# UBC-AWP/vision-sam3-yolo-lameless

Measured on AMD Instinct MI355X. Metric: frames/sec (whole node) for YOLO+SAM3+DINOv3 feature extraction, 1080p clips, higher is better.
Workload: dtype f16; 1 GPU; BASELINE cfg#5, dense schedule: fused per-frame path on a synthetic 5 s @ 30 fps 1080p clip (150 unique BGR frames resident in HBM): YOLOv8-l detect (letterbox 384x640, NMS, scale_boxes; f16 plan) -> SAM (Hiera-B+ image encoder + FPN at 1024x1024, box-prompted mask decoder, 1080p mask + statistics + contour features) + DINOv3 ViT-L/16 embed (224x224) on EVERY frame; per-frame records packed, gathe; parallelism=one clip per GPU, 1 GPU(s), one gather per step, streams=7

## Files before the change

include/lmx.h:

```cpp
#ifndef LMX_H
#define LMX_H
#include <stdint.h>
#ifdef __cplusplus
extern "C" {
#endif

#define LMX_VERSION 100

#define LMX_OK 0
#define LMX_EINVAL (-1)
#define LMX_EHIP (-2)

typedef void* lmx_stream_t;

int lmx_version(void);
const char* lmx_last_error(void);
int lmx_device_count(void);

enum { LMX_F16 = 0, LMX_F32 = 1 };
enum { LMX_ACT_NONE = 0, LMX_ACT_SILU = 1, LMX_ACT_GELU = 2 , LMX_ACT_RELU = 3,
       LMX_ACT_SWIGLU = 4  };

typedef struct {
  const void* A;
// ... 98 lines not shown
                        int a_off, int A, lmx_stream_t stream);
int lmx_k_scale_boxes(float* boxes, int total, float padx, float pady, float gain, float w, float h,
                      lmx_stream_t stream);

int lmx_k_split3(const float* x, int64_t ldx, int act, const void* res3, int64_t ldr, void* out3, int64_t ldo, int64_t rows,
                 int N, int g, int nsum, int64_t sum_stride, lmx_stream_t stream);
int lmx_k_maxpool5_x3(const void* src3, int64_t lds, void* dst3, int64_t ldd, int n, int H, int W, int C, lmx_stream_t stream);
int lmx_k_stem_conv_x3(const uint8_t* img, const float* w, const float* bias, void* out3, int n, int H, int W, int Cout,
                       lmx_stream_t stream);
int lmx_k_attention_f32(const float* q, int64_t ldq, const float* k, int64_t ldk, const float* v, int64_t ldv, float* o,
                        int64_t ldo, int B, int H, int Tq, int Tk, int hd, float scale, lmx_stream_t stream);
int lmx_k_hyper_mask_f32(const float* up, const float* hyper, float* logits, int n, int G, int C, int act, lmx_stream_t stream);

int lmx_k_pose_gather(const float* raw0, const float* raw1, const float* raw2, int64_t ldk, const int32_t* hw,
                      const float* strides, const int32_t* src, const int32_t* counts, int n, int max_det, int K, int ndim,
                      float padx, float pady, float gain, float w, float h, float* out, lmx_stream_t stream);

int lmx_k_im2col_u8(const uint8_t* img, const float* lut, void* out, int n, int rh, int rw, int IH, int IW, int KH,
                    int KW, int stride, int pad, int64_t ldo, lmx_stream_t stream);
int lmx_k_maxpool2(const void* src, int64_t lds, void* dst, int64_t ldd, int dtype, int n, int H, int W, int C,
                   lmx_stream_t stream);
int lmx_k_cast_f32_f16(const float* src, int64_t lds, void* dst, int64_t ldd, int64_t rows, int cols,
                       lmx_stream_t stream);

int lmx_k_add_bcast(const void* a, int a_dtype, int64_t lda, const float* b, int64_t ldb, int b_rows, void* out,
                    int out_dtype, int64_t ldo, int64_t rows, int D, lmx_stream_t stream);
int lmx_k_prompt_box(const float* boxes, int64_t ldb, float* sparse, int n, double sx, double sy, float S,
                     const float* gauss, const float* corner, int F, lmx_stream_t stream);
int lmx_k_hyper_mask(const void* up, const float* hyper, float* logits, int n, int G, int C, lmx_stream_t stream);
int lmx_k_mask_post(const float* logits, int n, int L, int T, int nh, int nw, int h, int w, uint8_t* mask,
                    int64_t* stats, float* workspace, lmx_stream_t stream);
int lmx_k_prompt_points(const float* points, const int32_t* labels, int Np, const float* boxes, int64_t ldb, float* sparse, int n,
                        double sx, double sy, float S, const float* gauss, const float* point_embed, const float* not_a_point,
                        const float* corner, int F, lmx_stream_t stream);
#define LMX_MASK_EMBED_PARAMS 4684
int lmx_k_mask_embed(const float* mask_input, const void* emb, int emb_dtype, int64_t lde, const float* params, float* keys,
                     int64_t ldk, int n, int G, lmx_stream_t stream);
int lmx_k_hyper_mask_multi(const void* up, const float* hyper, float* logits, int n, int M, int G, int C, lmx_stream_t stream);
int lmx_k_hyper_mask_multi_f32(const float* up, const float* hyper, float* logits, int n, int M, int G, int C, int act,
                               lmx_stream_t stream);
int lmx_k_mask_logits(const float* logits, int n, int L, int T, int nh, int nw, int h, int w, float* out, lmx_stream_t stream);

int lmx_k_mask_score(const float* logits, int n, int L, int T, int nh, int nw, int h, int w, double thr, double off,
                     const int32_t* idx, int64_t* out, lmx_stream_t stream);
int lmx_k_nms_boxes(const float* boxes, int64_t ldb, const float* scores, const uint8_t* valid, int n, double iou, int32_t* keep_out,
                    int32_t* count_out, void* workspace, lmx_stream_t stream);
// ... 15 lines not shown
```

vision-sam3-yolo-lameless_amd/csrc/sam.hip:

```cpp
#include "common.h"

namespace {

inline int grid_for(int64_t total, int block = 256) {
  int64_t g = (total + block - 1) / block;
  if (g > 256 * 8) g = 256 * 8;
  if (g < 1) g = 1;
  return (int)g;
}

template <int KW_T>
__global__ __launch_bounds__(256) void im2col_u8_kernel(const uint8_t* __restrict__ img, const float* __restrict__ lut,
                                                        half_t* __restrict__ out, int n, int rh, int rw, int OH, int OW, int KH,
                                                        int KW_rt, int stride, int pad, int64_t ldo) {
  __shared__ float lut_s[768];
  for (int i = threadIdx.x; i < 768; i += blockDim.x) lut_s[i] = lut[i];
  __syncthreads();
  const int KW = KW_T > 0 ? KW_T : KW_rt;
  const int chunks = (int)(ldo / 8);
  const int K = KH * KW * 3;
  const int64_t total = (int64_t)n * OH * OW * chunks;
  for (int64_t i = (int64_t)blockIdx.x * blockDim.x + threadIdx.x; i < total; i += (int64_t)gridDim.x * blockDim.x) {
    const int ck = (int)(i % chunks);
    const int64_t tok = i / chunks;
// ... 41 lines not shown
#pragma unroll
    for (int e = 0; e < VEC; ++e) {
      T t0 = a0[e] > a1[e] ? a0[e] : a1[e];
      T t1 = a2[e] > a3[e] ? a2[e] : a3[e];
      m[e] = t0 > t1 ? t0 : t1;
    }
    *reinterpret_cast<vec_t*>(dst + p * ldd + c) = m;
  }
}

__global__ __launch_bounds__(256) void cast_kernel(const float* __restrict__ src, int64_t lds, half_t* __restrict__ dst, int64_t ldd,
                                                   int64_t rows, int cols) {
  const int cc = cols / 4;
  const int64_t total = rows * cc;
  for (int64_t i = (int64_t)blockIdx.x * blockDim.x + threadIdx.x; i < total; i += (int64_t)gridDim.x * blockDim.x) {
    const int c = (int)(i % cc) * 4;
    const int64_t r = i / cc;
    const f32x4 v = *reinterpret_cast<const f32x4*>(src + r * lds + c);
    half4_t h = {(half_t)v[0], (half_t)v[1], (half_t)v[2], (half_t)v[3]};
    *reinterpret_cast<half4_t*>(dst + r * ldd + c) = h;
  }
}


template <int IN_DT, int OUT_DT>
__global__ __launch_bounds__(256) void add_bcast_kernel(const void* __restrict__ av, int64_t lda, const float* __restrict__ b,
                                                        int64_t ldb, int b_rows, void* __restrict__ out, int64_t ldo, int64_t rows,
                                                        int D) {
  const int cc = D / 4;
  const int64_t total = rows * cc;
  for (int64_t i = (int64_t)blockIdx.x * blockDim.x + threadIdx.x; i < total; i += (int64_t)gridDim.x * blockDim.x) {
    const int c = (int)(i % cc) * 4;
    const int64_t r = i / cc;
    f32x4 v;
    if (IN_DT == LMX_F32) {
      v = *reinterpret_cast<const f32x4*>(reinterpret_cast<const float*>(av) + r * lda + c);
    } else {
      const half4_t hv = *reinterpret_cast<const half4_t*>(reinterpret_cast<const half_t*>(av) + r * lda + c);
      v = f32x4{(float)hv[0], (float)hv[1], (float)hv[2], (float)hv[3]};
    }
    v += *reinterpret_cast<const f32x4*>(b + (r % b_rows) * ldb + c);
    if (OUT_DT == LMX_F32) {
      *reinterpret_cast<f32x4*>(reinterpret_cast<float*>(out) + r * ldo + c) = v;
    } else {
      half4_t h = {(half_t)v[0], (half_t)v[1], (half_t)v[2], (half_t)v[3]};
      *reinterpret_cast<half4_t*>(reinterpret_cast<half_t*>(out) + r * ldo + c) = h;
// ... 228 lines not shown
    hipLaunchKernelGGL((maxpool2_kernel<half_t, 8>), dim3(grid_for((int64_t)n * (H / 2) * (W / 2) * (C / 8))), dim3(256), 0, st,
                       reinterpret_cast<const half_t*>(src), lds, reinterpret_cast<half_t*>(dst), ldd, n, H, W, C);
  } else if (dtype == LMX_F32) {
    LMX_REQUIRE(C % 4 == 0 && lds % 4 == 0 && ldd % 4 == 0 && aligned16(src) && aligned16(dst), "lmx_k_maxpool2: f32 alignment");
    hipLaunchKernelGGL((maxpool2_kernel<float, 4>), dim3(grid_for((int64_t)n * (H / 2) * (W / 2) * (C / 4))), dim3(256), 0, st,
                       reinterpret_cast<const float*>(src), lds, reinterpret_cast<float*>(dst), ldd, n, H, W, C);
  } else {
    LMX_REQUIRE(false, "lmx_k_maxpool2: dtype %d", dtype);
  }
  return lmx_launch_check("maxpool2_kernel");
}

extern "C" int lmx_k_cast_f32_f16(const float* src, int64_t lds, void* dst, int64_t ldd, int64_t rows, int cols,
                                  lmx_stream_t stream) {
  LMX_REQUIRE(src && dst, "lmx_k_cast_f32_f16: null pointer");
  LMX_REQUIRE(rows > 0 && cols > 0 && cols % 4 == 0 && lds % 4 == 0 && ldd % 4 == 0 && lds >= cols && ldd >= cols,
              "lmx_k_cast_f32_f16: shape");
  LMX_REQUIRE(aligned16(src) && ((((uintptr_t)dst) & 7) == 0), "lmx_k_cast_f32_f16: alignment");
  hipLaunchKernelGGL(cast_kernel, dim3(grid_for(rows * (cols / 4))), dim3(256), 0, reinterpret_cast<hipStream_t>(stream), src, lds,
                     reinterpret_cast<half_t*>(dst), ldd, rows, cols);
  return lmx_launch_check("cast_kernel");
}

extern "C" int lmx_k_prompt_box(const float* boxes, int64_t ldb, float* sparse, int n, double sx, double sy, float S,
                                const float* gauss, const float* corner, int F, lmx_stream_t stream) {
  LMX_REQUIRE(boxes && sparse && gauss && corner && n > 0 && F > 0 && ldb >= 4 && S > 0.f, "lmx_k_prompt_box: arguments");
  hipLaunchKernelGGL(prompt_box_kernel, dim3((n * 2 * F + 255) / 256), dim3(256), 0, reinterpret_cast<hipStream_t>(stream), boxes, ldb,
                     sparse, n, sx, sy, S, gauss, corner, F);
  return lmx_launch_check("prompt_box_kernel");
}

extern "C" int lmx_k_add_bcast(const void* a, int a_dtype, int64_t lda, const float* b, int64_t ldb, int b_rows, void* out,
                               int out_dtype, int64_t ldo, int64_t rows, int D, lmx_stream_t stream) {
  LMX_REQUIRE(a && b && out, "lmx_k_add_bcast: null pointer");
  LMX_REQUIRE(rows > 0 && D > 0 && D % 4 == 0 && b_rows > 0 && lda >= D && ldb >= D && ldo >= D && lda % 4 == 0 && ldb % 4 == 0 &&
                  ldo % 4 == 0, "lmx_k_add_bcast: shape");
  LMX_REQUIRE(((((uintptr_t)a) & (a_dtype == LMX_F32 ? 15 : 7)) == 0) && aligned16(b) &&
                  ((((uintptr_t)out) & (out_dtype == LMX_F32 ? 15 : 7)) == 0), "lmx_k_add_bcast: alignment");
  hipStream_t st = reinterpret_cast<hipStream_t>(stream);
  const int g = grid_for(rows * (D / 4));
  if (a_dtype == LMX_F32 && out_dtype == LMX_F32)
    hipLaunchKernelGGL((add_bcast_kernel<LMX_F32, LMX_F32>), dim3(g), dim3(256), 0, st, a, lda, b, ldb, b_rows, out, ldo, rows, D);
  else if (a_dtype == LMX_F32 && out_dtype == LMX_F16)
    hipLaunchKernelGGL((add_bcast_kernel<LMX_F32, LMX_F16>), dim3(g), dim3(256), 0, st, a, lda, b, ldb, b_rows, out, ldo, rows, D);
  else if (a_dtype == LMX_F16 && out_dtype == LMX_F32)
    hipLaunchKernelGGL((add_bcast_kernel<LMX_F16, LMX_F32>), dim3(g), dim3(256), 0, st, a, lda, b, ldb, b_rows, out, ldo, rows, D);
// ... 59 lines not shown
```

vision-sam3-yolo-lameless_amd/lmx/_lib.py:

```python
import ctypes as C
import os

_HERE = os.path.dirname(os.path.abspath(__file__))
LIB_PATH = os.environ.get("LMX_LIB") or os.path.join(_HERE, "liblmx.so")


class LmxError(RuntimeError):
    pass


class GemmDesc(C.Structure):
    _fields_ = [
        ("A", C.c_void_p), ("W", C.c_void_p), ("bias", C.c_void_p), ("scale", C.c_void_p), ("res", C.c_void_p),
        ("C", C.c_void_p),
        ("lda", C.c_int64), ("ldc", C.c_int64), ("ldr", C.c_int64),
        ("M", C.c_int32), ("N", C.c_int32), ("K", C.c_int32),
        ("act", C.c_int32), ("out_dtype", C.c_int32), ("a_mode", C.c_int32),
        ("H", C.c_int32), ("W_", C.c_int32), ("Cin", C.c_int32), ("conv_stride", C.c_int32),
        ("Ho", C.c_int32), ("Wo", C.c_int32), ("res_rows", C.c_int32), ("a_rep", C.c_int32), ("split_k", C.c_int32), ("split_stride", C.c_int64),
        ("ln_out", C.c_void_p), ("ln_gamma", C.c_void_p), ("ln_beta", C.c_void_p), ("ld_ln", C.c_int64), ("ln_eps", C.c_float),
    ]


class AttnDesc(C.Structure):
# ... 32 lines not shown
    "lmx_k_pil_resize_h": (_I, [_VP, _VP, _I, _I, _I, _I, _VP, _VP, _I, _I, _VP]),
    "lmx_k_pil_resize_v": (_I, [_VP, _VP, _I, _I, _I, _I, _VP, _VP, _I, _VP]),
    "lmx_k_patchify_norm": (_I, [_VP, _VP, _I, _I, _I, _I, _I, _I, _I, _I, _I64, _VP, _VP]),
    "lmx_k_float_resize_patchify": (_I, [_VP, _VP, _I, _I, _I, _I, _I, _I, _I64, _VP, _VP, _I, _VP, _VP, _I, _I, _F, _VP, _I, _VP]),
    "lmx_k_assemble_tokens": (_I, [_VP, _VP, _VP, _VP, _I, _I, _I, _I, _VP]),
    "lmx_k_token_mean": (_I, [_VP, _I, _VP, _I, _I, _I, _VP]),
    "lmx_k_swiglu": (_I, [_VP, _I64, _VP, _I64, _I, _I, _VP]),
    "lmx_nms_workspace_bytes": (_I64, [_I, _I]),
    "lmx_k_nms": (_I, [_VP, _I, _I, _I, _F, _D, _I, _F, _VP, _VP, _VP, _VP, _VP, _VP, _VP]),
    "lmx_k_letterbox": (_I, [_VP, _VP, _I, _I, _I, _I, _I, _I, _I, _I, _I, _VP, _VP, _VP, _VP, _I, _VP]),
    "lmx_k_stem_conv": (_I, [_VP, _VP, _VP, _VP, _I, _I, _I, _I, _VP]),
    "lmx_k_split3": (_I, [_VP, _I64, _I, _VP, _I64, _VP, _I64, _I64, _I, _I, _I, _I64, _VP]),
    "lmx_k_maxpool5_x3": (_I, [_VP, _I64, _VP, _I64, _I, _I, _I, _I, _VP]),
    "lmx_k_stem_conv_x3": (_I, [_VP, _VP, _VP, _VP, _I, _I, _I, _I, _VP]),
    "lmx_k_attention_f32": (_I, [_VP, _I64, _VP, _I64, _VP, _I64, _VP, _I64, _I, _I, _I, _I, _I, _F, _VP]),
    "lmx_k_hyper_mask_f32": (_I, [_VP, _VP, _VP, _I, _I, _I, _I, _VP]),
    "lmx_k_maxpool5": (_I, [_VP, _I64, _VP, _I64, _I, _I, _I, _I, _VP]),
    "lmx_k_upsample2": (_I, [_VP, _I64, _VP, _I64, _I, _I, _I, _I, _VP]),
    "lmx_k_detect_decode": (_I, [_VP, _I64, _VP, _I, _I, _I, _I, _F, _I, _I, _VP]),
    "lmx_k_scale_boxes": (_I, [_VP, _I, _F, _F, _F, _F, _F, _VP]),
    "lmx_k_im2col_u8": (_I, [_VP, _VP, _VP, _I, _I, _I, _I, _I, _I, _I, _I, _I, _I64, _VP]),
    "lmx_k_maxpool2": (_I, [_VP, _I64, _VP, _I64, _I, _I, _I, _I, _I, _VP]),
    "lmx_k_cast_f32_f16": (_I, [_VP, _I64, _VP, _I64, _I64, _I, _VP]),
    "lmx_k_add_bcast": (_I, [_VP, _I, _I64, _VP, _I64, _I, _VP, _I, _I64, _I64, _I, _VP]),
    "lmx_h_mask_features": (_I, [_VP, _I, _I, _VP]),
    "lmx_h_iou_matrix": (_I, [_VP, _I, _VP, _I, _VP]),
    "lmx_h_assign": (_I, [_VP, _I, _I, _VP, _VP]),
    "lmx_contour_workspace_bytes": (_I64, [_I, _I, _I]),
    "lmx_k_contour_features": (_I, [_VP, _I, _I, _I, _VP, _VP, _VP]),
    "lmx_k_prompt_box": (_I, [_VP, _I64, _VP, _I, _D, _D, _F, _VP, _VP, _I, _VP]),
    "lmx_k_hyper_mask": (_I, [_VP, _VP, _VP, _I, _I, _I, _VP]),
    "lmx_k_mask_post": (_I, [_VP, _I, _I, _I, _I, _I, _I, _I, _VP, _VP, _VP, _VP]),
    "lmx_k_prompt_points": (_I, [_VP, _VP, _I, _VP, _I64, _VP, _I, _D, _D, _F, _VP, _VP, _VP, _VP, _I, _VP]),
    "lmx_k_mask_embed": (_I, [_VP, _VP, _I, _I64, _VP, _VP, _I64, _I, _I, _VP]),
    "lmx_k_hyper_mask_multi": (_I, [_VP, _VP, _VP, _I, _I, _I, _I, _VP]),
    "lmx_k_hyper_mask_multi_f32": (_I, [_VP, _VP, _VP, _I, _I, _I, _I, _I, _VP]),
    "lmx_k_mask_logits": (_I, [_VP, _I, _I, _I, _I, _I, _I, _I, _VP, _VP]),
    "lmx_k_mask_score": (_I, [_VP, _I, _I, _I, _I, _I, _I, _I, _D, _D, _VP, _VP, _VP]),
    "lmx_k_nms_boxes": (_I, [_VP, _I64, _VP, _VP, _I, _D, _VP, _VP, _VP, _VP]),
}

_lib = None


def load():
    global _lib
    if _lib is not None:
# ... 21 lines not shown
```

vision-sam3-yolo-lameless_amd/lmx/adapters.py:

```python
from pathlib import Path

import numpy as np
import torch

from . import checkpoints, dino, sam, sam_decoder, yolo
from .graphs import GraphedFn


def _device(device):
    if not torch.cuda.is_available():
        raise RuntimeError("lmx adapters need a GPU (liblmx has no CPU path)")
    return torch.device(device if device is not None else "cuda")


class Boxes:

    def __init__(self, xyxy, conf, cls):
        self.xyxy, self.conf, self.cls = xyxy, conf, cls

    def __len__(self):
        return int(self.xyxy.shape[0])

    def __getitem__(self, i):
        if isinstance(i, int):
# ... 150 lines not shown
    def apply_boxes(self, boxes, original_size):
        return self.apply_coords(np.asarray(boxes).reshape(-1, 2, 2), original_size).reshape(-1, 4)

    def apply_coords_torch(self, coords, original_size):
        old_h, old_w = original_size
        new_h, new_w = self.get_preprocess_shape(old_h, old_w, self.target_length)
        coords = coords.clone().to(torch.float)
        coords[..., 0] = coords[..., 0] * (new_w / old_w)
        coords[..., 1] = coords[..., 1] * (new_h / old_h)
        return coords

    def apply_boxes_torch(self, boxes, original_size):
        return self.apply_coords_torch(boxes.reshape(-1, 2, 2), original_size).reshape(-1, 4)


class LmxSamPredictor:

    def __init__(self, sam_model):
        self.model = sam_model
        self.encoder, self.decoder = sam_model.image_encoder, sam_model.mask_decoder
        self.device = sam_model.device
        self.transform = ResizeLongestSide(self.encoder.cfg.image)
        self.is_image_set = False
        self._g_encode = GraphedFn(lambda f: self.encoder.encode(f)["fpn"][2], clone_outputs=False)
        self._g_decode = {}

    @classmethod
    def from_parts(cls, encoder, decoder):
        m = type("LmxSamParts", (), {})()
        m.image_encoder, m.mask_decoder, m.device, m.cfg = encoder, decoder, encoder.device, encoder.cfg
        return cls(m)

    def reset_image(self):
        self.is_image_set = False
        self.features = None
        self.original_size = self.input_size = None

    def set_image(self, image, image_format="RGB"):
        a = np.asarray(image)
        if a.dtype != np.uint8 or a.ndim != 3 or a.shape[2] != 3:
            raise ValueError(f"set_image expects an HWC uint8 image, got {a.dtype} {a.shape}")
        if image_format not in ("RGB", "BGR"):
            raise ValueError(f"image_format must be 'RGB' or 'BGR', is {image_format}")
        if image_format == "BGR":
            a = a[..., ::-1]
        frames = torch.from_numpy(np.ascontiguousarray(a)[None]).to(self.device)
        self.original_size = tuple(a.shape[:2])
# ... 161 lines not shown
```

vision-sam3-yolo-lameless_amd/lmx/kernels.py:

```python
import ctypes as C
import os
import threading

import torch

from . import _lib
from ._lib import AttnDesc, GemmDesc, LmxError, check

F16, F32 = 0, 1
ACT_NONE, ACT_SILU, ACT_GELU, ACT_RELU, ACT_SWIGLU = 0, 1, 2, 3, 4
_DT = {torch.float16: F16, torch.float32: F32}


_tls = threading.local()


def _stream(dev):
    _tls.dev = dev
    return C.c_void_p(torch.cuda.current_stream(dev).cuda_stream)


def _ptr(t):
    return C.c_void_p(t.data_ptr()) if t is not None else C.c_void_p(0)

# ... 146 lines not shown
    out = torch.empty((n * OH * OW, ldo), dtype=torch.float16, device=img.device)
    check(_lib.load().lmx_k_im2col_u8(_ptr(img), _ptr(lut), _ptr(out), n, rh, rw, IH, IW, KH, KW, stride, pad, ldo,
                                      _stream(dev)), "lmx_k_im2col_u8")
    return out


def maxpool2(x, out):
    dev = _dev(x, out)
    n, H, W, Cc, ps = _nhwc(x, "maxpool2 x")
    no, Ho, Wo, Co, pso = _nhwc(out, "maxpool2 out")
    if (no, Ho, Wo, Co) != (n, H // 2, W // 2, Cc) or x.dtype != out.dtype:
        raise LmxError("maxpool2: shape/dtype mismatch")
    check(_lib.load().lmx_k_maxpool2(_ptr(x), ps, _ptr(out), pso, _DT[x.dtype], n, H, W, Cc, _stream(dev)), "lmx_k_maxpool2")
    return out


def cast_f16(x, out=None):
    dev = _dev(x, out)
    rows, cols, lds = _rows(x, "cast src")
    if out is None:
        out = torch.empty((rows, cols), dtype=torch.float16, device=x.device)
    check(_lib.load().lmx_k_cast_f32_f16(_ptr(x), lds, _ptr(out), out.stride(0), rows, cols, _stream(dev)),
          "lmx_k_cast_f32_f16")
    return out


def _nhwc(t, what):
    if t.dim() != 4 or t.stride(3) != 1:
        raise LmxError(f"{what}: expected NHWC with contiguous channels, got {tuple(t.shape)} / {t.stride()}")
    n, H, W, Cc = t.shape
    ps = t.stride(2)
    if t.stride(1) != W * ps or (n > 1 and t.stride(0) != H * W * ps):
        raise LmxError(f"{what}: not a channel slice of a dense NHWC buffer: strides {t.stride()}")
    return n, H, W, Cc, ps


def split_k_for(px_per_frame, N, K, cin):
    if N < 64 or N % 8 or cin % 32:
        return 1
    tiles1 = -(-px_per_frame // 256) * -(-N // 256)
    nk = K // 64
    s = min(8, nk // 8, 32 // tiles1)
    return s if s >= 2 else 1


def conv3x3(x, w, bias=None, act=ACT_SILU, stride=1, res=None, out=None, scale=None, out_dtype=torch.float16, split_k=1):
# ... 703 lines not shown
        return "fused attention half", rows * (8.0 * D * D + 256.0 * D), rows * D * (8 + (2 if args[0] else 0)), f"hiera_attn8 rows={rows} D={D} ln_inside={int(not args[0])}"
    if name == "lmx_k_hiera_attn4":
        n_, Gh, Gw, D = args[5], args[6], args[7], args[8]
        rows = n_ * Gh * Gw
        return "fused attention half", rows * (8.0 * D * D + 64.0 * D), rows * D * 10, f"hiera_attn4 rows={rows} D={D}"
    if name == "lmx_k_hiera_attn_pool":
        n_, Gh, Gw, Di, Do = args[4], args[5], args[6], args[7], args[8]
        rows = n_ * Gh * Gw
        keys = 64 if Di == 112 else 16
        return "fused attention half", rows * (8.0 * Di * Do + keys * Do + 0.5 * Do * Do), rows * (2 * Di + Do), f"hiera_attn_pool rows={rows} {Di}->{Do}"
    if name == "lmx_k_cast_f32_f16":
        rows, cols = args[4], args[5]
        return "streaming glue", 0.0, 6 * rows * cols, f"cast_f32_f16 rows={rows} cols={cols}"
    if name == "lmx_k_maxpool2":
        dt, n_, H, W, C_ = args[4], args[5], args[6], args[7], args[8]
        esz = 4 if dt == F32 else 2
        return "streaming glue", 0.0, esz * n_ * H * W * C_ * 5 // 4, f"maxpool2 n={n_} H={H} W={W} C={C_} dtype={dt}"
    if name == "lmx_k_upsample2":
        n_, H, W, C_ = args[4], args[5], args[6], args[7]
        return "streaming glue", 0.0, 2 * n_ * H * W * C_ * 5, f"upsample2 n={n_} H={H} W={W} C={C_}"
    if name == "lmx_k_add_bcast":
        a_dt, o_dt, rows, D = args[1], args[7], args[9], args[10]
        return "streaming glue", 0.0, rows * D * ((4 if a_dt == F32 else 2) + (4 if o_dt == F32 else 2)), f"add_bcast rows={rows} D={D}"
    if name == "lmx_k_rope":
        B, T, H, hd = args[2], args[3], args[4], args[5]
        return "streaming glue", 0.0, 2 * 2 * 2 * B * T * H * hd, f"rope B={B} T={T} H={H} hd={hd}"
    return "pre/post-processing and glue", 0.0, None, name


def _install_trace():
    global _raw_lib
    if _raw_lib is not None:
        return
    lib = _raw_lib = _lib.load()

    def make(name, fn):
        def traced(*args):
            if LAUNCH_TRACE is None:
                return fn(*args)
            cls, fl, by, key = _work(name, args)
            st = torch.cuda.current_stream(_tls.dev)
            e0, e1 = torch.cuda.Event(enable_timing=True), torch.cuda.Event(enable_timing=True)
            e0.record(st)
            rc = fn(*args)
            e1.record(st)
            LAUNCH_TRACE.append((cls, key, fl, by, e0, e1))
# ... 36 lines not shown
```

vision-sam3-yolo-lameless_amd/lmx/pipeline.py:

```python
import os

import torch

from . import dino, sam, sam_decoder, yolo
from . import kernels as K

DATA = os.path.join(os.path.dirname(os.path.abspath(__file__)), "data")


def stream_plan(n_chunks, max_streams=4, layout="lanes"):
    if layout not in ("lanes", "rr"):
        raise ValueError(f"stream layout {layout!r}: expected 'lanes' or 'rr'")
    k = max(3, min(2 + n_chunks, int(max_streams)))
    if layout == "rr":
        return k, 0, 1, [(2 + j) % k for j in range(n_chunks)]
    return k, 0, 1, [2 + j % (k - 2) for j in range(n_chunks)]


class FusedExtractor:
    def __init__(self, device="cuda", yolo_scale="l", weight_seeds=(7, 5, 3), yolo_bn=None):
        from . import weights

        self.device = torch.device(device)
        self.serial = bool(os.environ.get("LMX_SERIAL"))
# ... 67 lines not shown
            det_stream, emb_stream, sam_streams = main, main, [main] * len(chunks)
        else:
            n_pool, di, ei, si = stream_plan(max(1, len(chunks)), self.max_streams, self.stream_layout)
            pool = self._streams(n_pool)
            det_stream, emb_stream, sam_streams = pool[di], pool[ei], [pool[j] for j in si][:len(chunks)]
            for st in pool:
                st.wait_stream(main)
        empty = n == 0
        with torch.cuda.stream(det_stream):
            if empty:
                z = torch.zeros
                boxes, scores, cls, counts = (z((0, 300, 4), device=self.device), z((0, 300), device=self.device),
                                              z((0, 300), dtype=torch.int32, device=self.device), z((0,), dtype=torch.int32, device=self.device))
            else:
                boxes, scores, cls, src, counts = self.yolo.detect(frames, conf=conf, precision=precision)
            det_done = torch.cuda.Event()
            det_done.record(det_stream)
        with torch.cuda.stream(emb_stream):
            emb = (self.dino.embed_frames(emb_frames) if emb_frames.shape[0]
                   else torch.zeros((0, self.dino.cfg.hidden), dtype=torch.float32, device=self.device))
        masks, stats, ious, conts = [], [], [], []
        for i, st in zip(chunks, sam_streams):
            with torch.cuda.stream(st):
                enc = self.sam.encode(frames[i:i + sam_chunk], precision=precision)
                e2 = enc["fpn"][2]
                st.wait_event(det_done)
                d = self.decoder.predict(e2.view(-1, e2.shape[-1]), boxes[i:i + sam_chunk, 0, :], (h, w), rhw, precision=precision)
                conts.append(K.contour_features(d["mask"]))
            masks.append(d["mask"])
            stats.append(d["stats"])
            ious.append(d["iou"])
        for st in set(sam_streams + [det_stream, emb_stream]):
            if st is not main:
                main.wait_stream(st)
        if empty:
            mask = torch.zeros((0, h, w), dtype=torch.uint8, device=self.device)
            out = dict(boxes=boxes, scores=scores, cls=cls, counts=counts, embedding=emb,
                       mask_bits=torch.zeros((0, h, (w + 7) // 8), dtype=torch.uint8, device=self.device),
                       mask_stats=torch.zeros((0, 8), dtype=torch.int64, device=self.device),
                       mask_contour=torch.zeros((0, 8), dtype=torch.int64, device=self.device),
                       mask_iou=torch.zeros((0,), dtype=torch.float32, device=self.device))
        else:
            cat = (lambda ts: ts[0] if len(ts) == 1 else torch.cat(ts, 0))
            mask = cat(masks)
            out = dict(boxes=boxes, scores=scores, cls=cls, counts=counts, embedding=emb, mask_bits=K.pack_bits(mask),
                       mask_stats=cat(stats), mask_contour=cat(conts), mask_iou=cat(ious))
        if keep_byte_masks:
# ... 3 lines not shown
```

vision-sam3-yolo-lameless_amd/lmx/sam.py:

```python
import math
import os
from dataclasses import dataclass

import numpy as np
import torch

from . import kernels as K
from . import resample

SAM_PIXEL_MEAN = (123.675, 116.28, 103.53)
SAM_PIXEL_STD = (58.395, 57.12, 57.375)


@dataclass
class HieraConfig:
    hidden: int = 112
    blocks: tuple = (2, 3, 16, 3)
    dims: tuple = (112, 224, 448, 896)
    heads: tuple = (2, 4, 8, 16)
    windows: tuple = (8, 4, 14, 7)
    global_blocks: tuple = (12, 16, 20)
    pos_bkg: tuple = (14, 14)
    q_pool_stages: int = 3
    fpn_dim: int = 256
# ... 188 lines not shown
    kslot = np.array([16 * (2 * s_ + hb) + 4 * g + i for s_ in range(nks) for g in range(4) for hb in range(2) for i in range(4)])
    k15, k7 = (lambda r: r & 15), (lambda r: (r >> 1) & 7)
    imgs = []
    for ch in range(4 * D // 64):
        m1 = np.zeros((64, cols), np.float16)
        ok = kslot < D
        m1[:, ok] = w1[64 * ch: 64 * ch + 64][:, kslot[ok]].astype(np.float16)
        m2 = np.zeros((D, 64), np.float16)
        m2[:, :] = w2[:, 64 * ch + kslot[:64]].astype(np.float16)
        i1, i2 = _lds_image(m1, k15), _lds_image(m2, k7)
        if D <= 128:
            both = i1.copy()
            both[8192:8192 + D * 64] = i2[:D * 64]
            imgs.append(both)
        else:
            imgs += [i1, i2]
    z = np.zeros((D,), np.float32)
    bias = np.concatenate([b1, b2, g2, e2, gn if gn is not None else z, en if en is not None else z]).astype(np.float32)
    return np.stack(imgs), bias


class HieraEncoder:

    def __init__(self, cfg, state_dict, device="cuda", fused_mlp=True):
        self.cfg = cfg
        self.device = torch.device(device)
        self.fused_mlp = fused_mlp and not os.environ.get("LMX_NO_FUSED_MLP")
        dev = self.device
        sd = state_dict

        def t32(a):
            return torch.from_numpy(np.ascontiguousarray(a, dtype=np.float32)).to(dev)

        def t16(a):
            return t32(a).to(torch.float16).contiguous()

        w = np.transpose(sd["backbone.patch_embed.projection.weight"], (0, 2, 3, 1)).reshape(cfg.hidden, 147)
        self.k_pad = 152
        self.pe_w = t16(np.concatenate([w, np.zeros((cfg.hidden, self.k_pad - 147), np.float32)], 1))
        self.pe_b = t32(sd["backbone.patch_embed.projection.bias"])
        g = cfg.image // 4
        pe = torch.nn.functional.interpolate(torch.from_numpy(sd["backbone.pos_embed"]), size=(g, g), mode="bicubic")
        win = torch.from_numpy(sd["backbone.pos_embed_window"])
        pe = pe + win.tile([x // y for x, y in zip(pe.shape, win.shape)])
        self.pos = pe.permute(0, 2, 3, 1).reshape(g * g, cfg.hidden).contiguous().to(dev)
        self.grid0 = g
        self.blocks = []
        for i, (dim, dim_out, heads, win_, qs) in enumerate(cfg.block_plan()):
# ... 19 lines not shown
                blk["attn4"] = tuple(torch.from_numpy(a).to(dev) for a in pack_hiera_attn4(
                    np.asarray(sd[p + "attn.qkv.weight"], np.float32), np.asarray(qkv_b, np.float32),
                    np.asarray(sd[p + "attn.proj.weight"], np.float32), np.asarray(sd[p + "attn.proj.bias"], np.float32), heads))
            if qs and ((dim, dim_out, heads, win_) in ((112, 224, 4, 8), (224, 448, 8, 4))):
                blk["attnp"] = tuple(torch.from_numpy(a).to(dev) for a in pack_hiera_attn_pool(
                    np.asarray(sd[p + "proj.weight"], np.float32), np.asarray(sd[p + "proj.bias"], np.float32),
                    np.asarray(sd[p + "attn.qkv.weight"], np.float32), np.asarray(qkv_b, np.float32),
                    np.asarray(sd[p + "attn.proj.weight"], np.float32), np.asarray(sd[p + "attn.proj.bias"], np.float32), heads))
            blk["proj_ln"] = dim == dim_out == 448 and not qs and not (self.fused_mlp and dim_out in K.FUSED_MLP_WIDTHS)
            self.blocks.append(blk)
        for i, blk in enumerate(self.blocks):
            if blk["dim_out"] in (112, 224) and self.fused_mlp:
                p = f"backbone.blocks.{i}."
                nx = f"backbone.blocks.{i + 1}." if i + 1 < len(self.blocks) else None
                f32 = lambda k: np.asarray(sd[k], np.float32)
                blk["mlp_img"] = tuple(torch.from_numpy(a).to(dev) for a in pack_ln_mlp(
                    f32(p + "mlp.proj_in.weight"), f32(p + "mlp.proj_in.bias"), f32(p + "mlp.proj_out.weight"), f32(p + "mlp.proj_out.bias"),
                    f32(p + "layer_norm2.weight"), f32(p + "layer_norm2.bias"),
                    f32(nx + "layer_norm1.weight") if nx else None, f32(nx + "layer_norm1.bias") if nx else None))
        n = len(cfg.dims) - 1
        self.neck = [(t16(sd[f"neck.convs.{n - i}.weight"][:, :, 0, 0]), t32(sd[f"neck.convs.{n - i}.bias"])) for i in range(n + 1)]
        self.lut = t32(sam_norm_lut())
        self._tabs = {}

    def _tables(self, h, w):
        key = (h, w)
        if key not in self._tabs:
            nh, nw = resize_longest_side(h, w, self.cfg.image)
            dev = self.device

            def up(tab):
                b, k, ks = tab
                return (torch.from_numpy(b).to(dev), torch.from_numpy(k).to(dev), ks)

            th = up(resample.coeff_tables(w, nw, resample.BILINEAR)) if nw != w else None
            tv = up(resample.coeff_tables(h, nh, resample.BILINEAR)) if nh != h else None
            self._tabs[key] = (nh, nw, th, tv)
        return self._tabs[key]

    def preprocess(self, frames):
        n, h, w, _ = frames.shape
        nh, nw, th, tv = self._tables(h, w)
        img = K.pil_resize(frames, nw, nh, th, tv, swap_rb=False)
        S = self.cfg.image
        return img, K.im2col_u8(img, self.lut, S, S, 7, 7, 4, 3, self.k_pad)

    def trunk(self, patches, n):
        cfg = self.cfg
        g = self.grid0
        x = K.gemm(patches, self.pe_w, bias=self.pe_b, res=self.pos, res_rows=g * g, out_dtype=torch.float32)
        H = W = g
        stage_ends = set(int(v) for v in np.cumsum(cfg.blocks) - 1)
        stages, stages16 = [], []
        dev = x.device
        h_next = None
        for i, B in enumerate(self.blocks):
            dim, D, heads, qs = B["dim"], B["dim_out"], B["heads"], B["qs"]
            rows = n * H * W
            h2 = None
            if self._attn8(i, H, W):
                if B["attn8_ln"]:
                    K.hiera_attn8(x, B["attn8"], n, H, W, heads, ln=(B["g1"], B["b1"], cfg.eps))
                else:
                    K.hiera_attn8(x, B["attn8"], n, H, W, heads, h=h_next if h_next is not None else K.layernorm(x, B["g1"], B["b1"], cfg.eps))
            elif "attnp" in B and K.hiera_attn_pool_ok(dim, D, heads, B["win"], H, W, qs):
                x = K.hiera_attn_pool(h_next if h_next is not None else K.layernorm(x, B["g1"], B["b1"], cfg.eps), B["attnp"], n, H, W, heads, D)
                H, W = H // 2, W // 2
            elif "attn4" in B and K.hiera_attn4_ok(D, heads, B["win"], H, W, qs):
                K.hiera_attn4(h_next if h_next is not None else K.layernorm(x, B["g1"], B["b1"], cfg.eps), x, B["attn4"], n, H, W, heads)
            else:
                h = h_next if h_next is not None else K.layernorm(x, B["g1"], B["b1"], cfg.eps)
                if dim != D:
                    if qs and K.pooled_gemm_ok(rows, D):
                        sc = K.gemm(h, B["wp"], bias=B["bp"], out_dtype=torch.float32, pool_hw=(H, W))
                    else:
                        sc = K.gemm(h, B["wp"], bias=B["bp"], out_dtype=torch.float32)
                        if qs:
                            pooled = torch.empty((n, H // 2, W // 2, D), dtype=torch.float32, device=dev)
                            K.maxpool2(sc.view(n, H, W, D), pooled)
                            sc = pooled.view(-1, D)
                    res = sc
                else:
                    res = x
                x, H, W, h2 = self._attention_half(B, h, x, res, n, H, W)
            h_next = None
            x16 = None
            if D in K.FUSED_MLP_WIDTHS and self.fused_mlp:
                if i in stage_ends:
                    x16 = torch.empty((n * H * W, D), dtype=torch.float16, device=dev)
                nxt = None
                if i + 1 < len(self.blocks) and not (self._attn8(i + 1, H, W) and self.blocks[i + 1]["attn8_ln"]):
                    h_next = torch.empty((n * H * W, D), dtype=torch.float16, device=dev)
                    nxt = (self.blocks[i + 1]["g1"], self.blocks[i + 1]["b1"], h_next)
                if "mlp_img" in B and K.ln_mlp_img_ok(D, n * H * W):
                    K.ln_mlp_img(x, B["mlp_img"], cfg.eps, x16=x16, h_next=h_next)
                else:
                    K.ln_mlp(x, B["g2"], B["b2"], B["w1"], B["bb1"], B["w2"], B["bb2"], cfg.eps, x16=x16, next_ln=nxt)
            else:
                if h2 is None:
                    h2 = K.layernorm(x, B["g2"], B["b2"], cfg.eps)
                u = K.gemm(h2, B["w1"], bias=B["bb1"], act=K.ACT_GELU)
                K.gemm(u, B["w2"], bias=B["bb2"], res=x, out=x)
            if i in stage_ends:
                stages.append(x.view(n, H, W, D))
                stages16.append(x16)
                if i != len(self.blocks) - 1 and self.blocks[i + 1]["dim"] == self.blocks[i + 1]["dim_out"]:
                    x = x.clone()
        return stages, stages16

    def _attn8(self, i, H, W):
        B = self.blocks[i]
        return "attn8" in B and B["dim"] == B["dim_out"] and K.hiera_attn8_ok(B["dim_out"], B["heads"], B["win"], H, W, B["qs"])

    def _attention_half(self, B, h, x, res, n, H, W):
        D, heads, win, qs = B["dim_out"], B["heads"], B["win"], B["qs"]
        hd = D // heads
        rows = n * H * W
        dev = h.device
        Hq, Wq = H, W
        if qs and K.pooled_gemm_ok(rows, D):
            Hq, Wq = H // 2, W // 2
            q = K.gemm(h, B["wqkv"][:D], bias=B["bqkv"][:D], pool_hw=(H, W))
            kv = K.gemm(h, B["wqkv"][D:], bias=B["bqkv"][D:])
            k, v = kv[:, :D], kv[:, D:]
        else:
            qkv = K.gemm(h, B["wqkv"], bias=B["bqkv"])
            q, k, v = qkv[:, :D], qkv[:, D:2 * D], qkv[:, 2 * D:]
            if qs:
                Hq, Wq = H // 2, W // 2
                qp = torch.empty((n, Hq, Wq, D), dtype=torch.float16, device=dev)
                K.maxpool2(qkv.view(n, H, W, 3 * D)[..., :D], qp)
                q = qp.view(-1, D)
        a = torch.empty((n * Hq * Wq, D), dtype=torch.float16, device=dev)
        if win > 0:
            nW = -(-H // win) * -(-W // win)
            wq = win // 2 if qs else win
            K.attention(q, k, v, a, n * nW, heads, wq * wq, win * win, hd, hd ** -0.5,
                        window=dict(Gh=H, Gw=W, ws=win, q_stride=2 if qs else 1),
                        pad_k=B["padkv"][D:2 * D], pad_v=B["padkv"][2 * D:])
        else:
            K.attention(q, k, v, a, n, heads, Hq * Wq, H * W, hd, hd ** -0.5)
        xo = torch.empty((n * Hq * Wq, D), dtype=torch.float32, device=dev) if res is not x else x
        h2 = torch.empty((n * Hq * Wq, D), dtype=torch.float16, device=dev) if B["proj_ln"] else None
        K.gemm(a, B["wo"], bias=B["bo"], res=res, out=xo, ln_out=(h2, B["g2"], B["b2"], self.cfg.eps) if B["proj_ln"] else None)
        return xo, Hq, Wq, h2

    def fpn(self, stages, stages16=None):
        cfg = self.cfg
        nlev = len(stages) - 1
        feats, prev = [], None
        for i in range(nlev, -1, -1):
            s = stages[i]
            n, H, W, C = s.shape
            a = stages16[i] if stages16 and stages16[i] is not None else K.cast_f16(s.view(-1, C))
            w, b = self.neck[i]
            out = torch.empty((n, H, W, cfg.fpn_dim), dtype=torch.float16, device=s.device)
            if i not in cfg.fpn_top_down or i == nlev:
                K.gemm(a, w, bias=b, out=out.view(-1, cfg.fpn_dim))
            else:
                up = torch.empty((n, H, W, cfg.fpn_dim), dtype=torch.float16, device=s.device)
                K.upsample2(prev, up)
                K.gemm(a, w, bias=b, res=up.view(-1, cfg.fpn_dim), out=out.view(-1, cfg.fpn_dim))
            prev = out
            feats.append(out)
        return feats[-3:][::-1]

    def encode_patches(self, patches, n):
        stages, stages16 = self.trunk(patches, n)
        return dict(fpn=self.fpn(stages, stages16), stages=stages)

    def encode(self, frames, precision=None):
        img, patches = self.preprocess(frames)
        out = self.encode_patches(patches, frames.shape[0])
        out["resized"] = img
        return out


@dataclass
class SamVitConfig:
    hidden: int = 768
    layers: int = 12
    heads: int = 12
    mlp: int = 3072
    global_idx: tuple = (2, 5, 8, 11)
    window: int = 14
    patch: int = 16
    image: int = 1024
    out_ch: int = 256
    eps: float = 1e-6

    @property
    def grid(self):
        return self.image // self.patch


def sam_vit_b():
    return SamVitConfig()

# ... 132 lines not shown
                nW = (-(-g // ws)) ** 2
                K.attention(q, k, v, a, n * nW, H, ws * ws, ws * ws, hd, hd ** -0.5, window=dict(Gh=g, Gw=g, ws=ws, q_stride=1),
                            pad_k=L["padkv"][D:2 * D], pad_v=L["padkv"][2 * D:], rel_pos=(L["rh"], L["rw"]))
            lin(a, L["wo"], f"{i}.proj", bias=L["bo"], res=x, out=x)
            h2 = K.layernorm(x, L["g2"], L["b2"], cfg.eps)
            u = lin(h2, L["w1"], f"{i}.fc1", bias=L["bb1"], act=K.ACT_GELU)
            lin(u, L["w2"], f"{i}.fc2", bias=L["bb2"], res=x, out=x)
        y = lin(K.cast_f16(x), self.n1_w, "n1", out_dtype=torch.float32)
        y = K.layernorm(y, *self.n1_ln, 1e-6)
        y4 = y.view(n, g, g, cfg.out_ch)
        if exact:
            if "n2.hi" not in self._w2:
                w2 = self._split2("n2")
                Kc = w2.shape[1] // 2
                self._w2["n2.hi"], self._w2["n2.lo"] = w2[:, :Kc].contiguous(), w2[:, Kc:].contiguous()
            acc = K.conv3x3(y4, self._w2["n2.hi"], bias=None, act=K.ACT_NONE, out_dtype=torch.float32)
            acc = K.conv3x3(y4, self._w2["n2.lo"], bias=None, act=K.ACT_NONE, res=acc, out=acc)
            y = K.layernorm(acc.view(rows, cfg.out_ch), *self.n2_ln, 1e-6, out_dtype=torch.float32)
        else:
            y = K.conv3x3(y4, self.n2_w, bias=None, act=K.ACT_NONE)
            y = K.layernorm(y.view(rows, cfg.out_ch), *self.n2_ln, 1e-6)
        return y.view(n, g, g, cfg.out_ch)

    def encode(self, frames, precision=None):
        img, patches = self.preprocess(frames)
        return dict(fpn=[None, None, self.embed(patches, frames.shape[0], precision)], resized=img)
```

vision-sam3-yolo-lameless_amd/lmx/services/sam3_pipeline.py:

```python
import ctypes as C
import json
import traceback
from pathlib import Path

import numpy as np
import torch

from .. import _lib
from .. import kernels as K
from . import runtime as R

FEATURE_KEYS = ["mask_area", "area_ratio", "circularity", "aspect_ratio", "centroid_x", "centroid_y", "perimeter"]


def extract_segmentation_features(mask):
    m = np.ascontiguousarray(np.asarray(mask).astype(np.uint8))
    out = (C.c_double * 7)()
    rc = _lib.load().lmx_h_mask_features(m.ctypes.data_as(C.c_void_p), m.shape[0], m.shape[1], C.cast(out, C.c_void_p))
    if rc != 0:
        raise RuntimeError("lmx_h_mask_features failed")
    return {k: float(v) for k, v in zip(FEATURE_KEYS, out)}


def features_from_device(stats_row, contour_row, h, w):
# ... 128 lines not shown
                    if len(pend_ids) == self.batch:
                        flush()
            flush()
            await self.write_and_publish(video_id, self.results_from_features(ids, fps, total, feats))
        except Exception as e:
            print(f"Error in SAM3 pipeline for {video_id}: {e}")
            traceback.print_exc()

    async def start(self):
        await self.nats_client.connect()
        await self.nats_client.subscribe(self.config["nats"]["subjects"]["video_preprocessed"], self.process_video)


class HieraSegmenter:

    def __init__(self, encoder, decoder):
        self.encoder, self.decoder = encoder, decoder
        self.device = encoder.device

    def segment_records(self, frames, boxes):
        from .. import sam

        n, h, w, _ = frames.shape
        enc = self.encoder.encode(frames)
        e2 = enc["fpn"][2]
        d = self.decoder.predict(e2.view(-1, e2.shape[-1]), boxes, (h, w), sam.resize_longest_side(h, w, self.encoder.cfg.image))
        return dict(mask=d["mask"], stats=d["stats"], contour=K.contour_features(d["mask"]), iou=d["iou"])

    def segment(self, frames, boxes):
        return self.segment_records(frames, boxes)["mask"]


SamSegmenter = HieraSegmenter
```

Before: 690.2 frames/s.

## Skip padded rows in early Hiera stages and unused FPN levels

Adds a host planner that works out how many top patch rows of the letterboxed 1024x1024 input can affect outputs through the windowed blocks before the first global-attention block. Only that band is computed, and a cached table of constant rows, built once from padding, is joined in via a new band_join kernel. Encode also gains an 'embedding' mode that skips the high-resolution FPN levels the decoder never reads. The cost is a one-time table build that needs a device sync, so it cannot run during graph capture, plus more complex invariants about window alignment.

```diff
diff --git a/include/lmx.h b/include/lmx.h
--- a/include/lmx.h
+++ b/include/lmx.h
@@ -144,6 +144,9 @@
                    lmx_stream_t stream);
 int lmx_k_cast_f32_f16(const float* src, int64_t lds, void* dst, int64_t ldd, int64_t rows, int cols,
                        lmx_stream_t stream);
+int lmx_h_hiera_band(const int* window, const int* q_stride, int n_blocks, int grid, int nh, int nw, int* band);
+int lmx_k_band_join(const void* band, const void* table, void* out, int dtype, int n, int H, int Hb, int W, int D,
+                    lmx_stream_t stream);
 
 int lmx_k_add_bcast(const void* a, int a_dtype, int64_t lda, const float* b, int64_t ldb, int b_rows, void* out,
                     int out_dtype, int64_t ldo, int64_t rows, int D, lmx_stream_t stream);
diff --git a/vision-sam3-yolo-lameless_amd/csrc/sam.hip b/vision-sam3-yolo-lameless_amd/csrc/sam.hip
--- a/vision-sam3-yolo-lameless_amd/csrc/sam.hip
+++ b/vision-sam3-yolo-lameless_amd/csrc/sam.hip
@@ -87,6 +87,13 @@
   }
 }
 
+__global__ __launch_bounds__(256) void band_join_kernel(const u32x4* __restrict__ band, const u32x4* __restrict__ table,
+                                                        u32x4* __restrict__ out, int64_t ci, int64_t cb) {
+  const u32x4* bsrc = band + (int64_t)blockIdx.y * cb;
+  u32x4* o = out + (int64_t)blockIdx.y * ci;
+  for (int64_t i = (int64_t)blockIdx.x * blockDim.x + threadIdx.x; i < ci; i += (int64_t)gridDim.x * blockDim.x)
+    o[i] = i < cb ? bsrc[i] : table[i - cb];
+}
 
 template <int IN_DT, int OUT_DT>
 __global__ __launch_bounds__(256) void add_bcast_kernel(const void* __restrict__ av, int64_t lda, const float* __restrict__ b,
@@ -361,6 +368,59 @@
   return lmx_launch_check("cast_kernel");
 }
 
+extern "C" int lmx_h_hiera_band(const int* window, const int* q_stride, int n_blocks, int grid, int nh, int nw, int* band) {
+  LMX_REQUIRE(window && q_stride && band, "lmx_h_hiera_band: null pointer");
+  LMX_REQUIRE(n_blocks > 0 && grid > 0 && grid <= (1 << 20) && nh > 0 && nw > 0 && nh <= 4 * grid && nw <= 4 * grid,
+              "lmx_h_hiera_band: n_blocks=%d grid=%d nh=%d nw=%d", n_blocks, grid, nh, nw);
+  *band = 0;
+  if (nw < 4 * grid) return LMX_OK;
+  int64_t unit = 1, scale = 1;
+  int first_global = -1;
+  for (int i = 0; i < n_blocks; ++i) {
+    LMX_REQUIRE(window[i] >= 0 && (q_stride[i] == 0 || q_stride[i] == 1 || q_stride[i] == 2), "lmx_h_hiera_band: block %d: window=%d q_stride=%d",
+                i, window[i], q_stride[i]);
+    if (window[i] == 0) {
+      first_global = i;
+      break;
+    }
+    const int64_t pieces[2] = {window[i] * scale, q_stride[i] == 2 ? 2 * scale : scale};
+    for (int64_t p : pieces) {
+      int64_t a = unit, b = p;
+      while (b) {
+        const int64_t t = a % b;
+        a = b;
+        b = t;
+      }
+      unit = unit / a * p;
+    }
+    if (unit >= grid) return LMX_OK;
+    if (q_stride[i] == 2) scale *= 2;
+  }
+  if (first_global <= 0) return LMX_OK;
+  const int64_t d1 = (nh + 2) / 4 + 1;
+  const int64_t b = (d1 + unit - 1) / unit * unit;
+  if (b < grid) *band = (int)b;
+  return LMX_OK;
+}
+
+extern "C" int lmx_k_band_join(const void* band, const void* table, void* out, int dtype, int n, int H, int Hb, int W, int D,
+                               lmx_stream_t stream) {
+  LMX_REQUIRE(band && table && out, "lmx_k_band_join: null pointer");
+  LMX_REQUIRE(dtype == LMX_F16 || dtype == LMX_F32, "lmx_k_band_join: dtype %d", dtype);
+  LMX_REQUIRE(n > 0 && n <= 65535 && H > 0 && W > 0 && D > 0, "lmx_k_band_join: n=%d H=%d W=%d D=%d", n, H, W, D);
+  LMX_REQUIRE(Hb >= 1 && Hb <= H - 1, "lmx_k_band_join: Hb=%d outside 1 .. H - 1 = %d", Hb, H - 1);
+  const int64_t row_bytes = (int64_t)D * (dtype == LMX_F32 ? 4 : 2);
+  LMX_REQUIRE(row_bytes % 16 == 0, "lmx_k_band_join: a row of %lld bytes is not a multiple of 16", (long long)row_bytes);
+  LMX_REQUIRE(aligned16(band) && aligned16(table) && aligned16(out), "lmx_k_band_join: alignment");
+  const int64_t ci = (int64_t)H * W * (row_bytes / 16), cb = (int64_t)Hb * W * (row_bytes / 16);
+  int gx = grid_for(ci);
+  const int cap = 256 * 32 / n > 0 ? 256 * 32 / n : 1;
+  if (gx > cap) gx = cap;
+  hipLaunchKernelGGL(band_join_kernel, dim3(gx, n), dim3(256), 0, reinterpret_cast<hipStream_t>(stream),
+                     reinterpret_cast<const u32x4*>(band), reinterpret_cast<const u32x4*>(table), reinterpret_cast<u32x4*>(out), ci, cb);
+  return lmx_launch_check("band_join_kernel");
+}
+
 extern "C" int lmx_k_prompt_box(const float* boxes, int64_t ldb, float* sparse, int n, double sx, double sy, float S,
                                 const float* gauss, const float* corner, int F, lmx_stream_t stream) {
   LMX_REQUIRE(boxes && sparse && gauss && corner && n > 0 && F > 0 && ldb >= 4 && S > 0.f, "lmx_k_prompt_box: arguments");
diff --git a/vision-sam3-yolo-lameless_amd/lmx/_lib.py b/vision-sam3-yolo-lameless_amd/lmx/_lib.py
--- a/vision-sam3-yolo-lameless_amd/lmx/_lib.py
+++ b/vision-sam3-yolo-lameless_amd/lmx/_lib.py
@@ -78,7 +78,9 @@
     "lmx_k_im2col_u8": (_I, [_VP, _VP, _VP, _I, _I, _I, _I, _I, _I, _I, _I, _I, _I64, _VP]),
     "lmx_k_maxpool2": (_I, [_VP, _I64, _VP, _I64, _I, _I, _I, _I, _I, _VP]),
     "lmx_k_cast_f32_f16": (_I, [_VP, _I64, _VP, _I64, _I64, _I, _VP]),
-    "lmx_k_add_bcast": (_I, [_VP, _I, _I64, _VP, _I64, _I, _VP, _I, _I64, _I64, _I, _VP]),
+    "lmx_h_hiera_band": (_I, [C.POINTER(C.c_int), C.POINTER(C.c_int), _I, _I, _I, _I, C.POINTER(C.c_int)]),
+    "lmx_k_band_join": (_I, [_VP, _VP, _VP, _I, _I, _I, _I, _I, _I, _VP]),
+    "lmx_k_add_bcast":(_I, [_VP, _I, _I64, _VP, _I64, _I, _VP, _I, _I64, _I64, _I, _VP]),
     "lmx_h_mask_features": (_I, [_VP, _I, _I, _VP]),
     "lmx_h_iou_matrix": (_I, [_VP, _I, _VP, _I, _VP]),
     "lmx_h_assign": (_I, [_VP, _I, _I, _VP, _VP]),
diff --git a/vision-sam3-yolo-lameless_amd/lmx/adapters.py b/vision-sam3-yolo-lameless_amd/lmx/adapters.py
--- a/vision-sam3-yolo-lameless_amd/lmx/adapters.py
+++ b/vision-sam3-yolo-lameless_amd/lmx/adapters.py
@@ -196,7 +196,7 @@
         self.device = sam_model.device
         self.transform = ResizeLongestSide(self.encoder.cfg.image)
         self.is_image_set = False
-        self._g_encode = GraphedFn(lambda f: self.encoder.encode(f)["fpn"][2], clone_outputs=False)
+        self._g_encode = GraphedFn(lambda f: self.encoder.encode(f, outputs="embedding")["fpn"][2], clone_outputs=False)
         self._g_decode = {}
 
     @classmethod
diff --git a/vision-sam3-yolo-lameless_amd/lmx/kernels.py b/vision-sam3-yolo-lameless_amd/lmx/kernels.py
--- a/vision-sam3-yolo-lameless_amd/lmx/kernels.py
+++ b/vision-sam3-yolo-lameless_amd/lmx/kernels.py
@@ -192,6 +192,30 @@
         out = torch.empty((rows, cols), dtype=torch.float16, device=x.device)
     check(_lib.load().lmx_k_cast_f32_f16(_ptr(x), lds, _ptr(out), out.stride(0), rows, cols, _stream(dev)),
           "lmx_k_cast_f32_f16")
+    return out
+
+
+def hiera_band(windows, q_strides, grid, nh, nw):
+    nb = len(windows)
+    if nb != len(q_strides):
+        raise LmxError("hiera_band: windows and q_strides must be the same length")
+    band = C.c_int(0)
+    check(_lib.load().lmx_h_hiera_band((C.c_int * nb)(*windows), (C.c_int * nb)(*q_strides), nb, grid, nh, nw, C.byref(band)),
+          "lmx_h_hiera_band")
+    return band.value
+
+
+def band_join(band, table, H):
+    dev = _dev(band, table)
+    if band.dim() != 4 or table.dim() != 2 or not band.is_contiguous() or not table.is_contiguous():
+        raise LmxError("band_join: band must be contiguous [n, Hb, W, D] and table contiguous [(H - Hb) * W, D]")
+    n, Hb, W, D = band.shape
+    if band.dtype not in _DT or table.dtype != band.dtype or tuple(table.shape) != ((H - Hb) * W, D):
+        raise LmxError(f"band_join: table {table.dtype} {tuple(table.shape)} does not hold rows {Hb} .. {H - 1} of a {band.dtype} "
+                       f"[{H}, {W}, {D}] grid")
+    out = torch.empty((n, H, W, D), dtype=band.dtype, device=band.device)
+    check(_lib.load().lmx_k_band_join(_ptr(band), _ptr(table), _ptr(out), _DT[band.dtype], n, H, Hb, W, D, _stream(dev)),
+          "lmx_k_band_join")
     return out
 
 
@@ -941,6 +965,9 @@
     if name == "lmx_k_add_bcast":
         a_dt, o_dt, rows, D = args[1], args[7], args[9], args[10]
         return "streaming glue", 0.0, rows * D * ((4 if a_dt == F32 else 2) + (4 if o_dt == F32 else 2)), f"add_bcast rows={rows} D={D}"
+    if name == "lmx_k_band_join":
+        dt, n_, H, Hb, W, D = args[3:9]
+        return "streaming glue", 0.0, 2 * (4 if dt == F32 else 2) * n_ * H * W * D, f"band_join n={n_} H={H} Hb={Hb} W={W} D={D} dtype={dt}"
     if name == "lmx_k_rope":
         B, T, H, hd = args[2], args[3], args[4], args[5]
         return "streaming glue", 0.0, 2 * 2 * 2 * B * T * H * hd, f"rope B={B} T={T} H={H} hd={hd}"
diff --git a/vision-sam3-yolo-lameless_amd/lmx/pipeline.py b/vision-sam3-yolo-lameless_amd/lmx/pipeline.py
--- a/vision-sam3-yolo-lameless_amd/lmx/pipeline.py
+++ b/vision-sam3-yolo-lameless_amd/lmx/pipeline.py
@@ -113,7 +113,7 @@
         masks, stats, ious, conts = [], [], [], []
         for i, st in zip(chunks, sam_streams):
             with torch.cuda.stream(st):
-                enc = self.sam.encode(frames[i:i + sam_chunk], precision=precision)
+                enc = self.sam.encode(frames[i:i + sam_chunk], precision=precision, outputs="embedding")
                 e2 = enc["fpn"][2]
                 st.wait_event(det_done)
                 d = self.decoder.predict(e2.view(-1, e2.shape[-1]), boxes[i:i + sam_chunk, 0, :], (h, w), rhw, precision=precision)
diff --git a/vision-sam3-yolo-lameless_amd/lmx/sam.py b/vision-sam3-yolo-lameless_amd/lmx/sam.py
--- a/vision-sam3-yolo-lameless_amd/lmx/sam.py
+++ b/vision-sam3-yolo-lameless_amd/lmx/sam.py
@@ -1,5 +1,6 @@
 import math
 import os
+import threading
 from dataclasses import dataclass
 
 import numpy as np
@@ -234,8 +235,9 @@
 
 class HieraEncoder:
 
-    def __init__(self, cfg, state_dict, device="cuda", fused_mlp=True):
+    def __init__(self, cfg, state_dict, device="cuda", fused_mlp=True, band=True):
         self.cfg = cfg
+        self.band = band
         self.device = torch.device(device)
         self.fused_mlp = fused_mlp and not os.environ.get("LMX_NO_FUSED_MLP")
         dev = self.device
@@ -301,6 +303,8 @@
         self.neck = [(t16(sd[f"neck.convs.{n - i}.weight"][:, :, 0, 0]), t32(sd[f"neck.convs.{n - i}.bias"])) for i in range(n + 1)]
         self.lut = t32(sam_norm_lut())
         self._tabs = {}
+        self.first_global = next((i for i, B in enumerate(self.blocks) if B["win"] == 0), None)
+        self._bands, self._band_tabs, self._band_lock = {}, {}, threading.Lock()
 
     def _tables(self, h, w):
         key = (h, w)
@@ -317,23 +321,73 @@
             self._tabs[key] = (nh, nw, th, tv)
         return self._tabs[key]
 
-    def preprocess(self, frames):
+    def preprocess(self, frames, band=0):
         n, h, w, _ = frames.shape
         nh, nw, th, tv = self._tables(h, w)
         img = K.pil_resize(frames, nw, nh, th, tv, swap_rb=False)
         S = self.cfg.image
-        return img, K.im2col_u8(img, self.lut, S, S, 7, 7, 4, 3, self.k_pad)
-
-    def trunk(self, patches, n):
+        return img, K.im2col_u8(img, self.lut, 4 * band if band else S, S, 7, 7, 4, 3, self.k_pad)
+
+    def band_rows(self, nh, nw):
+        if (nh, nw) not in self._bands:
+            plan = self.cfg.block_plan()
+            self._bands[(nh, nw)] = K.hiera_band([p[3] for p in plan], [p[4] for p in plan], self.grid0, nh, nw)
+        return self._bands[(nh, nw)]
+
+    def _selection(self):
+        H = W = self.grid0
+        sel = []
+        for i, B in enumerate(self.blocks[:self.first_global]):
+            dim, D, heads, win, qs = B["dim"], B["dim_out"], B["heads"], B["win"], B["qs"]
+            sel.append((self._attn8(i, H, W), "attnp" in B and K.hiera_attn_pool_ok(dim, D, heads, win, H, W, qs),
+                        "attn4" in B and K.hiera_attn4_ok(D, heads, win, H, W, qs), "mlp_img" in B and K.ln_mlp_img_ok(D, H * W)))
+            if qs:
+                H, W = H // 2, W // 2
+        return tuple(sel)
+
+    def _band_table(self, frames, nh, nw, band):
+        key = (nh, nw, band, self._selection())
+        tab = self._band_tabs.get(key)
+        if tab is not None:
+            return tab
+        if torch.cuda.is_current_stream_capturing():
+            raise K.LmxError("HieraEncoder: the constant rows below the band are not built for this frame geometry, and a stream capture "
+                             "cannot build them (it needs a synchronisation): call encode() once before capturing")
+        with self._band_lock:
+            if key in self._band_tabs:
+                return self._band_tabs[key]
+            trace, K.LAUNCH_TRACE = K.LAUNCH_TRACE, None
+            try:
+                g = self.grid0
+                x, H, W, stages, stages16 = self.trunk(self.preprocess(frames[:1])[1], 1, until=self.first_global)
+
+                def below(t, Hs, Ws):
+                    return t.reshape(Hs, Ws, -1)[band * Hs // g:].reshape(-1, t.shape[-1]).clone()
+
+                tab = dict(x=below(x, H, W), stages=[below(s, *s.shape[1:3]) for s in stages],
+                           stages16=[below(s16, *s.shape[1:3]) if s16 is not None else None for s, s16 in zip(stages, stages16)])
+            finally:
+                K.LAUNCH_TRACE = trace
+            torch.cuda.current_stream(self.device).synchronize()
+            self._band_tabs[key] = tab
+        return tab
+
+    def trunk(self, patches, n, band=0, table=None, lowest=0, until=None):
         cfg = self.cfg
         g = self.grid0
-        x = K.gemm(patches, self.pe_w, bias=self.pe_b, res=self.pos, res_rows=g * g, out_dtype=torch.float32)
-        H = W = g
+        H, W = band or g, g
+        Hf = g
+        x = K.gemm(patches, self.pe_w, bias=self.pe_b, res=self.pos[:H * g], res_rows=H * g, out_dtype=torch.float32)
         stage_ends = set(int(v) for v in np.cumsum(cfg.blocks) - 1)
         stages, stages16 = [], []
         dev = x.device
         h_next = None
         for i, B in enumerate(self.blocks):
+            if i == until:
+                return x, H, W, stages, stages16
+            if band and i == self.first_global:
+                x = K.band_join(x.view(n, H, W, -1), table["x"], Hf).view(n * Hf * W, -1)
+                H, band, h_next = Hf, 0, None
             dim, D, heads, qs = B["dim"], B["dim_out"], B["heads"], B["qs"]
             rows = n * H * W
             h2 = None
@@ -362,10 +416,13 @@
                 else:
                     res = x
                 x, H, W, h2 = self._attention_half(B, h, x, res, n, H, W)
+            if qs:
+                Hf //= 2
             h_next = None
             x16 = None
+            keep = i in stage_ends and len(stages) >= lowest
             if D in K.FUSED_MLP_WIDTHS and self.fused_mlp:
-                if i in stage_ends:
+                if keep:
                     x16 = torch.empty((n * H * W, D), dtype=torch.float16, device=dev)
                 nxt = None
                 if i + 1 < len(self.blocks) and not (self._attn8(i + 1, H, W) and self.blocks[i + 1]["attn8_ln"]):
@@ -380,7 +437,14 @@
                     h2 = K.layernorm(x, B["g2"], B["b2"], cfg.eps)
                 u = K.gemm(h2, B["w1"], bias=B["bb1"], act=K.ACT_GELU)
                 K.gemm(u, B["w2"], bias=B["bb2"], res=x, out=x)
-            if i in stage_ends:
+            if i in stage_ends and not keep:
+                stages.append(None)
+                stages16.append(None)
+            elif i in stage_ends and band:
+                k = len(stages)
+                stages.append(K.band_join(x.view(n, H, W, D), table["stages"][k], Hf))
+                stages16.append(K.band_join(x16.view(n, H, W, D), table["stages16"][k], Hf).view(-1, D) if x16 is not None else None)
+            elif i in stage_ends:
                 stages.append(x.view(n, H, W, D))
                 stages16.append(x16)
                 if i != len(self.blocks) - 1 and self.blocks[i + 1]["dim"] == self.blocks[i + 1]["dim_out"]:
@@ -424,11 +488,11 @@
         K.gemm(a, B["wo"], bias=B["bo"], res=res, out=xo, ln_out=(h2, B["g2"], B["b2"], self.cfg.eps) if B["proj_ln"] else None)
         return xo, Hq, Wq, h2
 
-    def fpn(self, stages, stages16=None):
+    def fpn(self, stages, stages16=None, lowest=0):
         cfg = self.cfg
         nlev = len(stages) - 1
-        feats, prev = [], None
-        for i in range(nlev, -1, -1):
+        feats, prev = [None] * (nlev + 1), None
+        for i in range(nlev, lowest - 1, -1):
             s = stages[i]
             n, H, W, C = s.shape
             a = stages16[i] if stages16 and stages16[i] is not None else K.cast_f16(s.view(-1, C))
@@ -441,18 +505,24 @@
                 K.upsample2(prev, up)
                 K.gemm(a, w, bias=b, res=up.view(-1, cfg.fpn_dim), out=out.view(-1, cfg.fpn_dim))
             prev = out
-            feats.append(out)
-        return feats[-3:][::-1]
+            feats[i] = out
+        return feats[:3]
 
     def encode_patches(self, patches, n):
         stages, stages16 = self.trunk(patches, n)
         return dict(fpn=self.fpn(stages, stages16), stages=stages)
 
-    def encode(self, frames, precision=None):
-        img, patches = self.preprocess(frames)
-        out = self.encode_patches(patches, frames.shape[0])
-        out["resized"] = img
-        return out
+    def encode(self, frames, precision=None, outputs="all"):
+        if outputs not in ("all", "embedding"):
+            raise ValueError(f"outputs {outputs!r}: expected 'all' or 'embedding'")
+        lowest = 2 if outputs == "embedding" else 0
+        n, h, w, _ = frames.shape
+        nh, nw = self._tables(h, w)[:2]
+        band = self.band_rows(nh, nw) if self.band else 0
+        table = self._band_table(frames, nh, nw, band) if band else None
+        img, patches = self.preprocess(frames, band)
+        stages, stages16 = self.trunk(patches, n, band, table, lowest)
+        return dict(fpn=self.fpn(stages, stages16, lowest), stages=stages, resized=img)
 
 
 @dataclass
@@ -631,6 +701,6 @@
             y = K.layernorm(y.view(rows, cfg.out_ch), *self.n2_ln, 1e-6)
         return y.view(n, g, g, cfg.out_ch)
 
-    def encode(self, frames, precision=None):
+    def encode(self, frames, precision=None, outputs="all"):
         img, patches = self.preprocess(frames)
         return dict(fpn=[None, None, self.embed(patches, frames.shape[0], precision)], resized=img)
diff --git a/vision-sam3-yolo-lameless_amd/lmx/services/sam3_pipeline.py b/vision-sam3-yolo-lameless_amd/lmx/services/sam3_pipeline.py
--- a/vision-sam3-yolo-lameless_amd/lmx/services/sam3_pipeline.py
+++ b/vision-sam3-yolo-lameless_amd/lmx/services/sam3_pipeline.py
@@ -174,7 +174,7 @@
         from .. import sam
 
         n, h, w, _ = frames.shape
-        enc = self.encoder.encode(frames)
+        enc = self.encoder.encode(frames, outputs="embedding")
         e2 = enc["fpn"][2]
         d = self.decoder.predict(e2.view(-1, e2.shape[-1]), boxes, (h, w), sam.resize_longest_side(h, w, self.encoder.cfg.image))
         return dict(mask=d["mask"], stats=d["stats"], contour=K.contour_features(d["mask"]), iou=d["iou"])
```

Measured after the change: 788.6 frames/s (median of 6 runs). +14.3%, better.
